# abcqmars/audio-visual-sepatation-in-visual-agnostic-situtation

Measured on AMD Instinct MI355X. Metric: mixtures/sec (train step, 2-src MUSIC shape), higher is better.
Workload: dtype f32; 1 GPU; full HIP path, AV train step: 2-source mix, batch 64/GPU (BASELINE configs[2] shape), 65535-sample waveforms -> HIP STFT 1022/256 -> 256x256 log-freq tiles, 3x224^2 frames/source, unet7+hidsep(sig)+resnet18dilated, BCE, SGD; f32 arithmetic; visual trunk on this library (no MIOpen kernel in the step); global_batch=64, parallelism=dp1

## Files before the change

### audio-visual-sepatation-in-visual-agnostic-situtation_amd/csrc/conv3x3.hip

```cpp
#include <stdlib.h>

#include "halo_kernel.h"
#include "conv_families.h"

__global__ void c3_pack_kernel(const float* __restrict__ w, float* __restrict__ out, int Cout, int Cin, int rows, int ld,
                               int mode) {
  long long i = (long long)blockIdx.x * blockDim.x + threadIdx.x;
  if (i >= (long long)rows * ld) return;
  int row = (int)(i / ld), col = (int)(i % ld);
  int parity = row & 1, q = row >> 1, tap = q % 9, ch = 2 * (q / 9) + parity;
  float v = 0.f;
  if (mode == 0) {
    if (ch < Cin && col < Cout) v = w[((long long)col * Cin + ch) * 9 + tap];
  } else {
    if (ch < Cout && col < Cin) v = w[((long long)ch * Cin + col) * 9 + (8 - tap)];
  }
  out[i] = v;
}

static bool c3_flat_enabled(int algo) { return !(algo & AVSEP_ALGO_NO_FLAT); }
static bool c3_flat(const avsep_conv_desc* d) {
  return !d->up2x && d->C0 == d->Cin && c3_flat_width(d->H, d->W, d->dil) > 0 && (long long)d->N * d->H * d->W < 0x7fffffffLL &&
         c3_flat_enabled(d->algo);
}
// ... 96 lines not shown
  } else {
    int per = Cout * 4, cls = row / per, rr = row % per;
    int parity = rr & 1, q = rr >> 1, tap = q % 4, ch = 2 * (q / 4) + parity;
    int ph = cls >> 1, pw = cls & 1, th = tap >> 1, tw = tap & 1;
    int kh = ph ? 2 - 2 * th : 3 - 2 * th, kw = pw ? 2 - 2 * tw : 3 - 2 * tw;
    if (ch < Cout && col < Cin) v = w[((long long)ch * Cin + col) * 16 + kh * 4 + kw];
  }
  out[i] = v;
}

bool c4_applicable(const avsep_conv_desc* d, int mode) {
  if (!(d->KH == 4 && d->KW == 4 && d->stride == 2 && d->pad == 1 && d->dil == 1) || d->up2x) return false;
  if (d->Wo < 16 || d->Ho < 4 || d->N > 65535) return false;
  if (mode == 0) return d->Cin % 2 == 0 && d->C0 % 2 == 0 && d->Cout >= 32;
  return d->Cout % 8 == 0 && d->Cin >= 32 && (d->H & 1) == 0 && (d->W & 1) == 0;
}
size_t c4_packed_floats(const avsep_conv_desc* d, int mode) {
  int rows = (mode == 0 ? d->Cin : d->Cout) * 16, ld = roundup(mode == 0 ? d->Cout : d->Cin, 128);
  return (size_t)rows * ld;
}
int c4_pack(const avsep_conv_desc* d, const float* w, float* packed, int mode, hipStream_t st) {
  int rows = (mode == 0 ? d->Cin : d->Cout) * 16, ld = roundup(mode == 0 ? d->Cout : d->Cin, 128);
  long long total = (long long)rows * ld;
  hipLaunchKernelGGL(c4_pack_kernel, dim3(cdiv(total, 256)), dim3(256), 0, st, w, packed, d->Cout, d->Cin, rows, ld, mode);
  AVSEP_LAUNCH_CHECK();
  return AVSEP_OK;
}

template <int KS_, int S_, int CK_>
static int c4_launch(C3Args& a, hipStream_t st) {
  const bool wide = a.Wo >= 32;
  a.tilesX = cdiv(a.Wo, wide ? 32 : 16);
  a.tilesY = cdiv(a.Ho, wide ? 4 : 8);
  const bool narrow = c3_narrow_rule(a.Cout, (long long)cdiv(a.Cout, 128) * a.tilesX * a.tilesY * c3_plan_n(a), false);
  a.gridM = cdiv(a.Cout, narrow ? 64 : 128);
  dim3 grid((unsigned)((long long)a.gridM * a.tilesX * a.tilesY * a.N));
  if (wide && !narrow) hipLaunchKernelGGL((conv3x3_kernel<4, 32, 128, false, KS_, S_, 1, CK_>), grid, dim3(256), 0, st, a);
  else if (wide) hipLaunchKernelGGL((conv3x3_kernel<4, 32, 64, false, KS_, S_, 1, CK_>), grid, dim3(256), 0, st, a);
  else if (!narrow) hipLaunchKernelGGL((conv3x3_kernel<8, 16, 128, false, KS_, S_, 1, CK_>), grid, dim3(256), 0, st, a);
  else hipLaunchKernelGGL((conv3x3_kernel<8, 16, 64, false, KS_, S_, 1, CK_>), grid, dim3(256), 0, st, a);
  AVSEP_LAUNCH_CHECK();
  return AVSEP_OK;
}

int c4_fwd(const avsep_conv_desc* d, const float* wp, const float* bias, float* y, double* stats, void*, size_t,
           hipStream_t st) {
  C3Args a{};
  a.N = d->N; a.planN = d->plan_n; a.algo = d->algo; a.Cin = d->Cin; a.H = d->H; a.W = d->W; a.Cout = d->Cout;
  a.C0 = d->C0; a.C1 = d->Cin - d->C0; a.act0 = d->act0; a.act1 = d->act1; a.up2x = 0;
  a.Hs = d->H; a.Ws = d->W;
  a.x0 = d->x0; a.x1 = d->x1; a.sc0 = d->scale0; a.sh0 = d->shift0; a.sc1 = d->scale1; a.sh1 = d->shift1;
  a.wp = wp; a.wp_ld = roundup(d->Cout, 128); a.out = y; a.bias = bias; a.stats = stats;
  a.Ho = d->Ho; a.Wo = d->Wo; a.padh = a.padw = 1; a.os = 1; a.ooh = a.oow = 0; a.OHs = d->Ho; a.OWs = d->Wo;
  return c4_launch<4, 2, 2>(a, st);
}

int c4_dgrad(const avsep_conv_desc* d, const float* wp, const float* dy, float* dx, const avsep_act_bwd*, void*, size_t,
             hipStream_t st) {
  const int ld = roundup(d->Cin, 128);
  for (int cls = 0; cls < 4; ++cls) {
    const int ph = cls >> 1, pw = cls & 1;
    C3Args a{};
    a.N = d->N; a.planN = d->plan_n; a.algo = d->algo; a.Cin = d->Cout; a.H = d->Ho; a.W = d->Wo; a.Cout = d->Cin;
    a.C0 = d->Cout; a.C1 = 0; a.Hs = d->Ho; a.Ws = d->Wo;
    a.x0 = dy; a.wp = wp + (size_t)cls * d->Cout * 4 * ld; a.wp_ld = ld; a.out = dx;
    a.Ho = d->H / 2; a.Wo = d->W / 2; a.padh = ph ? 0 : 1; a.padw = pw ? 0 : 1;
    a.os = 2; a.ooh = ph; a.oow = pw; a.OHs = d->H; a.OWs = d->W;
    int rc = c4_launch<2, 1, 8>(a, st);
    if (rc) return rc;
  }
  return AVSEP_OK;
}

int c1x4_stft_fwd(const float* xt, const float* wp, float* out, int R, int NH, int hop, int cout, int frames,
                  hipStream_t st) {
  C3Args a{};
  a.N = 1; a.Cin = hop; a.H = R; a.W = NH; a.Cout = cout;
  a.C0 = hop; a.C1 = 0; a.Hs = R; a.Ws = NH;
  a.x0 = xt; a.wp = wp; a.wp_ld = roundup(cout, 128); a.out = out;
  a.Ho = R; a.Wo = frames; a.padh = a.padw = 0; a.os = 1; a.ooh = a.oow = 0; a.OHs = R; a.OWs = frames;
  a.tilesX = cdiv(frames, 32); a.tilesY = cdiv(R, 4); a.gridM = cdiv(cout, 128);
  dim3 grid((unsigned)((long long)a.gridM * a.tilesX * a.tilesY));
  hipLaunchKernelGGL((conv3x3_kernel<4, 32, 128, false, 1, 1, 1, 4, 1, 4>), grid, dim3(256), 0, st, a);
  AVSEP_LAUNCH_CHECK();
  return AVSEP_OK;
}

struct W3Args {
  int N, Cin, H, W, Cout, Ho, Wo;
  int C0, C1, act0, act1, up2x, Hs, Ws;
  float rh, rw;
  const float *x0, *x1, *sc0, *sh0, *sc1, *sh1;
  const float* dy;
  float* out;
  int tilesX, tilesY, gridM, gridC, tiles_per_split;
  int tapmajor;
};

constexpr int W3_CC = 32;

__device__ __forceinline__ float w3_src(const W3Args& a, int n, int c, int hs, int ws) {
  float v;
  if (c < a.C0) {
    v = a.x0[(((long long)n * a.C0 + c) * a.Hs + hs) * a.Ws + ws];
    if (a.sc0) v = fmaf(v, a.sc0[c], a.sh0[c]);
    v = act_apply(v, a.act0);
  } else {
    int c1 = c - a.C0;
    v = a.x1[(((long long)n * a.C1 + c1) * a.Hs + hs) * a.Ws + ws];
    if (a.sc1) v = fmaf(v, a.sc1[c1], a.sh1[c1]);
    v = act_apply(v, a.act1);
  }
  return v;
}

template <int TH, int TW, int PW, int MAXT, int TAP0, int NTAP, int DIL = 1, int S = 1>
__device__ __forceinline__ void w3_mfma_tile(const float* Ap, const float* Bp, f32x16 (&acc)[MAXT]) {
#pragma unroll 1
  for (int py = 0; py < TH; ++py) {
    const float* ar = Ap + py * TW;
    const float* br = Bp + py * S * PW;
    float av[2], bv[2][NTAP];
    av[0] = ar[0];
#pragma unroll
    for (int j = 0; j < NTAP; ++j) bv[0][j] = br[(((TAP0 + j) / 3) * PW + (TAP0 + j) % 3) * DIL];
#pragma unroll 4
    for (int px = 0; px < TW; px += 2) {
      const int cur = (px >> 1) & 1;
      if (px + 2 < TW) {
        av[cur ^ 1] = ar[px + 2];
#pragma unroll
        for (int j = 0; j < NTAP; ++j) bv[cur ^ 1][j] = br[(((TAP0 + j) / 3) * PW + (TAP0 + j) % 3) * DIL + (px + 2) * S];
      }
      __builtin_amdgcn_sched_barrier(0);
#pragma unroll
      for (int j = 0; j < NTAP; ++j) acc[j] = __builtin_amdgcn_mfma_f32_32x32x2f32(av[cur], bv[cur][j], acc[j], 0, 0, 0);
      __builtin_amdgcn_sched_barrier(0);
    }
  }
}

template <int TH, int TW, bool UP2X, int BM, int DIL = 1, bool A2 = false, int S = 1>
__global__ __launch_bounds__(512, 2) void wgrad3x3_kernel(W3Args a) {
  static_assert(!(UP2X && DIL != 1), "the fused upsample path is undilated");
  static_assert(S == 1 || (DIL == 1 && !UP2X), "stride 2: plain 3x3 / pad 1");
  constexpr int NPIX = TH * TW, PH = (TH - 1) * S + 2 * DIL + 1, PW = (TW - 1) * S + 2 * DIL + 1;
  constexpr int PS = (PH * PW) | 1;
  constexpr int LDA = NPIX + 1;
  constexpr int NT = 512;
  constexpr int NP = W3_CC * PH * PW, PE = (NP + NT - 1) / NT;
  constexpr int NA4 = BM * NPIX / 4, AE = NA4 / NT;
  static_assert(NA4 % NT == 0, "A tile must split evenly");
  __shared__ float smem[2 * W3_CC * PS + 2 * BM * LDA];
  float (*Ps)[W3_CC * PS] = reinterpret_cast<float (*)[W3_CC * PS]>(smem);
  float (*As)[BM * LDA] = reinterpret_cast<float (*)[BM * LDA]>(smem + 2 * W3_CC * PS);

  const int tid = threadIdx.x, lane = tid & 63, wave = tid >> 6, li = lane & 31, lk = lane >> 5;
  const int t_ = xcd_remap(blockIdx.x, gridDim.x), per_split_ = a.gridM * a.gridC;
  const int split = t_ / per_split_, lin_ = t_ % per_split_;
  const int mt = lin_ % a.gridM, ct = lin_ / a.gridM;
  const int m0 = mt * BM, c0 = ct * W3_CC;
  const int tiles_img = a.tilesX * a.tilesY, tiles_all = tiles_img * a.N;
  const int t_begin = split * a.tiles_per_split, t_end = min(tiles_all, t_begin + a.tiles_per_split);
  const long long HW = (long long)a.Ho * a.Wo;

  constexpr int RB = BM / 32, MAXT = (BM == 128) ? 5 : 3;
// ... 268 lines not shown
```

### audio-visual-sepatation-in-visual-agnostic-situtation_amd/csrc/conv_families.h

```cpp
#pragma once
#include "common.h"

typedef bool conv_applicable_fn(const avsep_conv_desc* d, int mode);
typedef size_t conv_packed_floats_fn(const avsep_conv_desc* d, int mode);
typedef int conv_pack_fn(const avsep_conv_desc* d, const float* w, float* packed, int mode, hipStream_t st);
typedef size_t conv_workspace_fn(const avsep_conv_desc* d, int mode);
typedef void conv_variant_fn(const avsep_conv_desc* d, int mode, char* buf, size_t cap);
typedef int conv_fwd_fn(const avsep_conv_desc* d, const float* wp, const float* bias, float* y, double* stats, void* ws,
                        size_t ws_bytes, hipStream_t st);
typedef int conv_dgrad_fn(const avsep_conv_desc* d, const float* wp, const float* dy, float* dx, const avsep_act_bwd* e,
                          void* ws, size_t ws_bytes, hipStream_t st);
typedef int conv_wgrad_fn(const avsep_conv_desc* d, const float* dy, float* dw, float* dbias, float* ws, hipStream_t st);

static inline int igemm_packed_ld(const avsep_conv_desc* d, int mode) { return roundup(mode == 0 ? d->Cout : d->Cin, 128); }

int splitk_combine(const float* ws, long long slab, int S, const avsep_conv_desc* d, const float* bias, float* y, double* stats,
                   hipStream_t st);
int reduce_slabs(const float* ws, float* out, long long n, int S, hipStream_t st);
int reduce_slabs_strided(const float* ws, float* out, long long n, int S, long long stride, hipStream_t st);

conv_applicable_fn smallco_applicable;  conv_workspace_fn smallco_workspace_bytes;  conv_fwd_fn smallco_fwd;  conv_wgrad_fn smallco_wgrad;
conv_applicable_fn smallci_applicable;  conv_packed_floats_fn smallci_packed_floats;  conv_pack_fn smallci_pack;  conv_dgrad_fn smallci_dgrad;

conv_applicable_fn head_applicable;  conv_workspace_fn head_workspace_bytes;  conv_fwd_fn head_fwd;  conv_wgrad_fn head_wgrad;
size_t head_dgrad_workspace_floats(const avsep_conv_desc* d);
int head_dgrad(const avsep_conv_desc* d, const float* w, const float* dy, float* g0, float* g1, const float* mean1,
               const float* invstd1, double* bstats1, int acc0, float* ws, hipStream_t st);

conv_applicable_fn bf_applicable;  conv_packed_floats_fn bf_packed_floats;  conv_pack_fn bf_pack;  conv_workspace_fn bf_workspace_bytes;
conv_fwd_fn bf_fwd;  conv_dgrad_fn bf_dgrad;  conv_variant_fn bf_variant;
bool bf_out_b16(const avsep_conv_desc* d, int mode);

conv_applicable_fn w4_applicable;  conv_packed_floats_fn w4_packed_floats;  conv_pack_fn w4_pack;
conv_fwd_fn w4_fwd;  conv_dgrad_fn w4_dgrad;  conv_variant_fn w4_variant;

conv_applicable_fn wn_applicable;  conv_packed_floats_fn wn_packed_floats;  conv_pack_fn wn_pack;  conv_fwd_fn wn_fwd;  conv_dgrad_fn wn_dgrad;

conv_applicable_fn c3_applicable;  conv_packed_floats_fn c3_packed_floats;  conv_pack_fn c3_pack;
conv_fwd_fn c3_fwd;  conv_dgrad_fn c3_dgrad;  conv_variant_fn c3_variant;
conv_applicable_fn c4_applicable;  conv_packed_floats_fn c4_packed_floats;  conv_pack_fn c4_pack;
conv_fwd_fn c4_fwd;  conv_dgrad_fn c4_dgrad;  conv_variant_fn c4_variant;
conv_applicable_fn w3_applicable;  conv_workspace_fn w3_workspace_bytes;  conv_wgrad_fn w3_wgrad;
void c3_variant_text(int M, int Ho, int Wo, long long planN, bool flat, bool quantise, char* buf, size_t cap);
int w3_reduce(const float* ws, float* dw, long long P, int splits, hipStream_t st);
int c1x4_stft_fwd(const float* xt, const float* wp, float* out, int R, int NH, int hop, int cout, int frames, hipStream_t st);

struct C3Args;
int c3_flat_width(int H, int W, int dil);
int c3_flat_launch(C3Args& a, int dil, hipStream_t st);

conv_applicable_fn cm_applicable;  conv_packed_floats_fn cm_packed_floats;  conv_pack_fn cm_pack;
conv_fwd_fn cm_fwd;  conv_dgrad_fn cm_dgrad;  conv_variant_fn cm_variant;

conv_applicable_fn wbn_applicable;  conv_workspace_fn wbn_workspace_bytes;  conv_wgrad_fn wbn_wgrad;  conv_variant_fn wbn_variant;
int b16_channel_sum(const void* x, int N, int C, int HW, double* acc, float* out, hipStream_t st);

conv_applicable_fn x4_applicable;  conv_workspace_fn x4_workspace_bytes;  conv_wgrad_fn x4_wgrad;  conv_variant_fn x4_variant;

conv_applicable_fn ww_applicable;  conv_workspace_fn ww_workspace_bytes;  conv_wgrad_fn ww_wgrad;
conv_applicable_fn w4d_applicable;  conv_workspace_fn w4d_workspace_bytes;  conv_wgrad_fn w4d_wgrad;

conv_applicable_fn scw_applicable;  conv_workspace_fn scw_workspace_bytes;  conv_wgrad_fn scw_wgrad;
```

### audio-visual-sepatation-in-visual-agnostic-situtation_amd/csrc/halo_kernel.h

```cpp
#pragma once
#include "common.h"

struct C3Args {
  int N, Cin, H, W, Cout;
  int C0, C1, act0, act1, up2x, Hs, Ws;
  float rh, rw;
  const float *x0, *x1, *sc0, *sh0, *sc1, *sh1;
  const float* wp;
  int wp_ld;
  float* out;
  const float* bias;
  double* stats;
  int tilesX, tilesY, gridM;
  int Ho, Wo;
  int padh, padw;
  int os, ooh, oow;
  int OHs, OWs;
  int kts;
  long long slab;
  int planN;
  int algo;
  int out16;
  int xs2;
};
static inline long long c3_plan_n(const C3Args& a) { return a.planN > 0 ? a.planN : a.N; }
static inline bool c3_narrow_rule(int cout, long long wg128, bool quantise) {
  return cout <= 64 || wg128 < 384 || (quantise && wg128 < 1024 && wg128 * 5 < ((wg128 + 255) / 256) * 256 * 4);
}

constexpr int C3_CK = 4;

__device__ __forceinline__ float c3_src(const C3Args& a, int n, int c, int hs, int ws) {
  float v;
  if (c < a.C0) {
    v = a.x0[(((long long)n * a.C0 + c) * a.Hs + hs) * a.Ws + ws];
    if (a.sc0) v = fmaf(v, a.sc0[c], a.sh0[c]);
    v = act_apply(v, a.act0);
  } else {
    int c1 = c - a.C0;
    v = a.x1[(((long long)n * a.C1 + c1) * a.Hs + hs) * a.Ws + ws];
    if (a.sc1) v = fmaf(v, a.sc1[c1], a.sh1[c1]);
    v = act_apply(v, a.act1);
  }
  return v;
}

template <int TH, int TW, int BM, bool UP2X, int KS = 3, int S = 1, int DIL = 1, int CK = 4, int KH_ = KS, int KW_ = KS,
          int FW = 0, bool ZF = false>
__global__ __launch_bounds__(256) void conv3x3_kernel(C3Args a) {
  constexpr bool FLAT = FW > 0;
  static_assert(!ZF || (!FLAT && !UP2X), "zero fill: rectangular tiles");
  static_assert(!FLAT || (S == 1 && !UP2X && (KH_ & 1) && (KW_ & 1)), "flat tiles: stride 1, odd taps, no fused upsample");
  constexpr int NT = KH_ * KW_, C3_KT = CK * NT, C3_CK = CK;
  constexpr int PADH = DIL * (KH_ - 1) / 2, PADW = DIL * (KW_ - 1) / 2;
  constexpr int F_NR = (FW + 126 + (FLAT ? FW : 1)) / (FLAT ? FW : 1);
  constexpr int F_NC = 127 / (FLAT ? FW * FW : 1) + 1;
  constexpr int PH = FLAT ? F_NR + F_NC * PADH + 2 * PADH : (TH - 1) * S + (KH_ - 1) * DIL + 1;
  constexpr int PWR = FLAT ? FW + 2 * PADW : (TW - 1) * S + (KW_ - 1) * DIL + 1;
  constexpr int PW = (S == 2) ? (PWR + 1) / 2 * 2 : PWR, PWH = PW / 2, PS = PH * PW;
  constexpr int LDA = BM + 4;
  constexpr int NPATCH = C3_CK * PS;
  constexpr int PE = (NPATCH + 255) / 256;
  constexpr int A4 = BM / 4, NA4 = C3_KT * A4, AE = (NA4 + 255) / 256;
  constexpr int WTM = BM / 2, TM = WTM / 32;
  __shared__ __attribute__((aligned(16))) float As[2][C3_KT][LDA];
  __shared__ float Ps[2][NPATCH];

  const int tid = threadIdx.x, lane = tid & 63, wave = tid >> 6;
  const int wm = wave >> 1, wn = wave & 1, li = lane & 31, lk = lane >> 5;
  int t = xcd_remap(blockIdx.x, gridDim.x);
  const int mt = t % a.gridM; t /= a.gridM;
  const int tx = t % a.tilesX; t /= a.tilesX;
  const int ty = t % a.tilesY;
  const int n = t / a.tilesY;
  const int h0 = ty * TH, w0 = tx * TW, m0 = mt * BM;
  const int f_HW = a.H * a.W, f_Hp = a.H + PADH, f_P = a.N * f_HW;
  const int p0 = tx * 128;
  const int vr0 = FLAT ? (p0 / f_HW) * f_Hp + (p0 % f_HW) / FW : 0;

  const bool has0 = a.sc0 != nullptr, has1 = a.sc1 != nullptr;
  const long long sHW = (long long)a.Hs * a.Ws;
  f32x4 areg[AE];
  const float* aptr[AE];
  int a_lds[AE];
#pragma unroll
  for (int e = 0; e < AE; ++e) {
    int idx = min(tid + 256 * e, NA4 - 1);
    int row = idx / A4, c4 = idx % A4;
    aptr[e] = a.wp + (long long)row * a.wp_ld + m0 + c4 * 4;
    a_lds[e] = row * LDA + c4 * 4;
  }
  const long long a_step = (long long)C3_KT * a.wp_ld;

  constexpr int NRAW = UP2X ? 4 : 1;
  float praw[PE][NRAW], psc[PE], psh[PE], plh[UP2X ? PE : 1], plw[UP2X ? PE : 1];
  const float* pptr[PE][NRAW];
  long long poff1[PE][NRAW];
  int p_cc[PE];
  int p_lds[S == 2 ? PE : 1];
  unsigned pok = 0;
#pragma unroll
  for (int e = 0; e < PE; ++e) {
    int idx = min(tid + 256 * e, NPATCH - 1);
    int cc = idx / PS, r = (idx % PS) / PW, col = idx % PW;
    int gh = h0 * S - a.padh + r, gw = w0 * S - a.padw + col;
    int ne = n;
    if constexpr (FLAT) {
      const int vr = vr0 - PADH + r;
      ne = vr >= 0 ? vr / f_Hp : a.N;
      gh = vr >= 0 ? vr % f_Hp : -1;
      gw = col - PADW;
      if (ne >= a.N) { ne = a.N - 1; gh = -1; }
    }
    if constexpr (S == 2) p_lds[e] = cc * PS + r * PW + (col & 1) * PWH + (col >> 1);
    bool ok = (PE * 256 == NPATCH || tid + 256 * e < NPATCH) && (unsigned)gh < (unsigned)a.H && (unsigned)gw < (unsigned)a.W;
    int ghc = min(max(gh, 0), a.H - 1), gwc = min(max(gw, 0), a.W - 1);
    long long o[NRAW];
    if constexpr (!UP2X) {
      o[0] = ((long long)ghc * a.Ws + gwc) << a.xs2;
    } else {
      float fh = a.rh * (float)ghc, fw = a.rw * (float)gwc;
      int hh0 = (int)fh, ww0 = (int)fw;
      int hh1 = hh0 + (hh0 < a.Hs - 1), ww1 = ww0 + (ww0 < a.Ws - 1);
      plh[e] = fh - (float)hh0;
      plw[e] = fw - (float)ww0;
      o[0] = (long long)hh0 * a.Ws + ww0; o[1] = (long long)hh0 * a.Ws + ww1;
      o[2] = (long long)hh1 * a.Ws + ww0; o[3] = (long long)hh1 * a.Ws + ww1;
    }
#pragma unroll
    for (int q = 0; q < NRAW; ++q) {
      pptr[e][q] = a.x0 + ((long long)ne * a.C0 + cc) * sHW + o[q];
      poff1[e][q] = ((long long)ne * a.C1 + cc) * sHW + o[q];
    }
    p_cc[e] = cc;
    pok |= (unsigned)ok << e;
  }
  const long long p_step = (long long)C3_CK * sHW;
  const int kt_switch = a.C0 / C3_CK;
  bool cur_has = has0;
  const float *scp = a.sc0, *shp = a.sh0;

  auto issue = [&](int kt) __attribute__((always_inline)) {
    if (kt == kt_switch && a.C1 > 0) {
#pragma unroll
      for (int e = 0; e < PE; ++e)
#pragma unroll
        for (int q = 0; q < NRAW; ++q) pptr[e][q] = a.x1 + poff1[e][q];
      cur_has = has1;
      scp = a.sc1;
      shp = a.sh1;
    }
#pragma unroll
    for (int e = 0; e < AE; ++e) {
      areg[e] = *reinterpret_cast<const f32x4*>(aptr[e]);
      aptr[e] += a_step;
    }
#pragma unroll
    for (int e = 0; e < PE; ++e) {
#pragma unroll
      for (int q = 0; q < NRAW; ++q) {
        praw[e][q] = *pptr[e][q];
        pptr[e][q] += p_step;
      }
      if (cur_has) {
        psc[e] = scp[p_cc[e]];
        psh[e] = shp[p_cc[e]];
      }
    }
    if (cur_has) {
      scp += C3_CK;
      shp += C3_CK;
    }
// ... 155 lines not shown
```

### audio-visual-sepatation-in-visual-agnostic-situtation_amd/csrc/stft.hip

```cpp
#include "common.h"
#include "conv_families.h"
#include "stft_parts.h"

static inline int bins_of(int n_fft) { return n_fft / 2 + 1; }

extern "C" size_t avsep_stft_basis_floats(int32_t n_fft, int32_t inverse) {
  if (n_fft < 2 || (n_fft & 1)) return 0;
  int b2 = 2 * bins_of(n_fft);
  return inverse ? (size_t)roundup(b2, 32) * roundup(n_fft, 128) : (size_t)roundup(n_fft, 32) * roundup(b2, 128);
}

__global__ void stft_basis_kernel(int n_fft, int bins, int rows, int ld, int inverse, float* __restrict__ out) {
  long long i = (long long)blockIdx.x * blockDim.x + threadIdx.x;
  if (i >= (long long)rows * ld) return;
  int row = (int)(i / ld), col = (int)(i % ld);
  int n = inverse ? col : row, m = inverse ? row : col;
  float v = 0.f;
  if (n < n_fft && m < 2 * bins) {
    int bin = m < bins ? m : m - bins;
    double win = 0.5 - 0.5 * cos(2.0 * M_PI * (double)n / (double)n_fft);
    long long prod = ((long long)bin * n) % n_fft;
    double ang = 2.0 * M_PI * (double)prod / (double)n_fft;
    double tr = (m < bins) ? cos(ang) : -sin(ang);
    if (inverse) {
// ... 1 lines not shown
      if (m >= bins && (bin == 0 || bin == n_fft / 2)) ck = 0.0;
      tr *= ck / (double)n_fft;
    }
    v = (float)(win * tr);
  }
  out[i] = v;
}

extern "C" int avsep_stft_basis(int32_t n_fft, float* fwd_basis, float* inv_basis, avsep_stream_t stream) {
  if (n_fft < 2 || (n_fft & 1)) return AVSEP_ERR_ARG;
  int bins = bins_of(n_fft), b2 = 2 * bins;
  if (fwd_basis) {
    int rows = roundup(n_fft, 32), ld = roundup(b2, 128);
    hipLaunchKernelGGL(stft_basis_kernel, dim3(cdiv((long long)rows * ld, 256)), dim3(256), 0, (hipStream_t)stream, n_fft,
                       bins, rows, ld, 0, fwd_basis);
    AVSEP_LAUNCH_CHECK();
  }
  if (inv_basis) {
    int rows = roundup(b2, 32), ld = roundup(n_fft, 128);
    hipLaunchKernelGGL(stft_basis_kernel, dim3(cdiv((long long)rows * ld, 256)), dim3(256), 0, (hipStream_t)stream, n_fft,
                       bins, rows, ld, 1, inv_basis);
    AVSEP_LAUNCH_CHECK();
  }
  return AVSEP_OK;
}

__global__ __launch_bounds__(256) void stft_pad_kernel(const float* __restrict__ wav, int L, int pad, int reflect,
                                                       float* __restrict__ out) {
  const int r = blockIdx.y, Lp = L + 2 * pad;
  for (int i = blockIdx.x * 256 + threadIdx.x; i < Lp; i += gridDim.x * 256) {
    int j = i - pad;
    float v = 0.f;
    if (j >= 0 && j < L) v = wav[(long long)r * L + j];
    else if (reflect) {
      if (j < 0) j = -j;
      if (j >= L) j = 2 * (L - 1) - j;
      if (j >= 0 && j < L) v = wav[(long long)r * L + j];
    }
    out[(long long)r * Lp + i] = v;
  }
}

__global__ __launch_bounds__(256) void stft_pad_t_kernel(const float* __restrict__ wav, int L, int pad, int reflect, int hop,
                                                         int R, int NH, float* __restrict__ xt) {
  extern __shared__ float tile[];
  const int r = blockIdx.y, j0 = blockIdx.x * 32, Lp = L + 2 * pad, ldt = hop + 1;
  for (int i = threadIdx.x; i < 32 * hop; i += 256) {
    const int jj = i / hop, c = i % hop, pos = (j0 + jj) * hop + c;
    float v = 0.f;
    if (pos < Lp) {
      int s = pos - pad;
      if (s >= 0 && s < L) v = wav[(long long)r * L + s];
      else if (reflect) {
        if (s < 0) s = -s;
        if (s >= L) s = 2 * (L - 1) - s;
        if (s >= 0 && s < L) v = wav[(long long)r * L + s];
      }
    }
    tile[jj * ldt + c] = v;
  }
  __syncthreads();
  for (int i = threadIdx.x; i < 32 * hop; i += 256) {
    const int c = i / 32, jj = i % 32;
    if (j0 + jj < NH) xt[((long long)c * R + r) * NH + j0 + jj] = tile[jj * ldt + c];
  }
}

__global__ void stft_basis_repack_kernel(const float* __restrict__ basis, int n_fft, int hop, int ntap, int ld,
                                         float* __restrict__ out) {
  long long i = (long long)blockIdx.x * blockDim.x + threadIdx.x;
  if (i >= (long long)hop * ntap * ld) return;
  const int row = (int)(i / ld), col = (int)(i % ld);
  const int par = row & 1, q = row >> 1, j = q % ntap, c = 2 * (q / ntap) + par, k = hop * j + c;
  out[i] = k < n_fft ? basis[(long long)k * ld + col] : 0.f;
}

__global__ __launch_bounds__(256) void stft_magphase_kernel(const float* __restrict__ spec, int bins, int frames, int R,
                                                            int co_major, float* __restrict__ mag,
                                                            float* __restrict__ phase) {
  const int r = blockIdx.y;
  const long long n = (long long)bins * frames;
  for (long long i = (long long)blockIdx.x * 256 + threadIdx.x; i < n; i += (long long)gridDim.x * 256) {
    float a, b;
    if (co_major) {
      const long long m = i / frames, f = i % frames;
      a = spec[(m * R + r) * frames + f];
      b = spec[((bins + m) * R + r) * frames + f];
    } else {
      a = spec[(long long)r * 2 * n + i];
      b = spec[(long long)r * 2 * n + n + i];
    }
    mag[(long long)r * n + i] = sqrtf(a * a + b * b);
    if (phase) phase[(long long)r * n + i] = atan2f(b, a);
  }
}


static bool stft_fast(int R, int L, int n_fft, int hop) {
  return n_fft > 3 * hop && n_fft <= 4 * hop && (hop & 3) == 0 && hop <= 1024 && 1 + L / hop >= 32 && R >= 1;
}
extern "C" size_t avsep_stft_workspace_bytes(int32_t R, int32_t L, int32_t n_fft, int32_t hop) {
  if (R <= 0 || L <= 0 || n_fft < 2 || hop <= 0) return 0;
  size_t frames = 1 + L / hop;
  size_t spec = (size_t)R * 2 * bins_of(n_fft) * frames;
  if (stft_fast(R, L, n_fft, hop))
    return ((size_t)hop * R * (frames + 3) + (size_t)hop * 4 * roundup(2 * bins_of(n_fft), 128) + spec) * sizeof(float);
  return ((size_t)R * (L + n_fft) + spec) * sizeof(float);
}

bool stft_fast_path(int R, int L, int n_fft, int hop) { return stft_fast(R, L, n_fft, hop); }

int stft_repack_basis(const float* basis, int n_fft, int hop, float* wp, hipStream_t st) {
  const int ld = roundup(2 * bins_of(n_fft), 128);
  hipLaunchKernelGGL(stft_basis_repack_kernel, dim3(cdiv((long long)hop * 4 * ld, 256)), dim3(256), 0, st, basis, n_fft, hop,
                     4, ld, wp);
  AVSEP_LAUNCH_CHECK();
  return AVSEP_OK;
}

int stft_pad_gemm(const float* wav, int R, int L, int n_fft, int hop, int reflect, const float* basis, float* stage, float* spec,
                  hipStream_t st) {
  const int pad = n_fft / 2, Lp = L + 2 * pad, bins = bins_of(n_fft), frames = 1 + L / hop;
  if (stft_fast(R, L, n_fft, hop)) {
    const int NH = frames + 3;
    hipLaunchKernelGGL(stft_pad_t_kernel, dim3(cdiv(NH, 32), R), dim3(256), (size_t)32 * (hop + 1) * sizeof(float), st, wav, L,
                       pad, reflect, hop, R, NH, stage);
    AVSEP_LAUNCH_CHECK();
    return c1x4_stft_fwd(stage, basis, spec, R, NH, hop, 2 * bins, frames, st);
  }
  hipLaunchKernelGGL(stft_pad_kernel, dim3(min(cdiv(Lp, 256), 1024), R), dim3(256), 0, st, wav, L, pad, reflect, stage);
  AVSEP_LAUNCH_CHECK();
  avsep_conv_desc d{};
  d.N = R; d.Cin = 1; d.H = 1; d.W = Lp; d.Cout = 2 * bins; d.Ho = 1; d.Wo = frames;
  d.KH = 1; d.KW = n_fft; d.stride = hop; d.pad = 0; d.dil = 1; d.C0 = 1; d.x0 = stage;
  return avsep_conv2d_fwd(&d, basis, nullptr, spec, nullptr, nullptr, 0, (avsep_stream_t)st);
}

int istft_gemm(const float* spec, int R, int n_fft, int frames, const float* inv_basis, float* td, hipStream_t st) {
  avsep_conv_desc d{};
  d.N = R; d.Cin = 2 * bins_of(n_fft); d.H = 1; d.W = frames; d.Cout = n_fft; d.Ho = 1; d.Wo = frames;
  d.KH = 1; d.KW = 1; d.stride = 1; d.pad = 0; d.dil = 1; d.C0 = d.Cin; d.x0 = spec;
  return avsep_conv2d_fwd(&d, inv_basis, nullptr, td, nullptr, nullptr, 0, (avsep_stream_t)st);
}

extern "C" int avsep_stft_mag(const float* wav, int32_t R, int32_t L, int32_t n_fft, int32_t hop, int32_t reflect,
                              const float* basis, float* mag, float* phase, void* workspace, size_t workspace_bytes,
                              avsep_stream_t stream) {
  if (!wav || !basis || !mag || R <= 0 || R > 65535 || L <= n_fft / 2 || n_fft < 2 || (n_fft & 1) || hop <= 0)
    return AVSEP_ERR_ARG;
  if (!workspace || workspace_bytes < avsep_stft_workspace_bytes(R, L, n_fft, hop)) return AVSEP_ERR_WORKSPACE;
  const int pad = n_fft / 2, Lp = L + 2 * pad, bins = bins_of(n_fft), frames = 1 + L / hop;
  hipStream_t st = (hipStream_t)stream;
  const bool fast = stft_fast(R, L, n_fft, hop);
  float* stage = (float*)workspace;
  const float* b = basis;
  float* spec;
  if (fast) {
    float* wp = stage + (size_t)hop * R * (frames + 3);
    spec = wp + (size_t)hop * 4 * roundup(2 * bins, 128);
    int rc = stft_repack_basis(basis, n_fft, hop, wp, st);
    if (rc) return rc;
    b = wp;
  } else {
    spec = stage + (size_t)R * Lp;
  }
  int rc = stft_pad_gemm(wav, R, L, n_fft, hop, reflect, b, stage, spec, st);
  if (rc) return rc;
  long long n = (long long)bins * frames;
  hipLaunchKernelGGL(stft_magphase_kernel, dim3((int)min((n + 255) / 256, (long long)1024), R), dim3(256), 0, st, spec, bins,
                     frames, R, fast ? 1 : 0, mag, phase);
  AVSEP_LAUNCH_CHECK();
  return AVSEP_OK;
}

__global__ __launch_bounds__(256) void istft_spec_kernel(const float* __restrict__ mag, const float* __restrict__ phase,
                                                         long long n, float* __restrict__ spec) {
  const int r = blockIdx.y;
  for (long long i = (long long)blockIdx.x * 256 + threadIdx.x; i < n; i += (long long)gridDim.x * 256) {
    float m = mag[(long long)r * n + i], p = phase[(long long)r * n + i];
    float s, c;
    sincosf(p, &s, &c);
    spec[(long long)r * 2 * n + i] = m * c;
    spec[(long long)r * 2 * n + n + i] = m * s;
  }
}

__global__ __launch_bounds__(256) void istft_ola_kernel(const float* __restrict__ td, int n_fft, int hop, int frames,
                                                        int out_len, float* __restrict__ wav) {
  const int r = blockIdx.y, pad = n_fft / 2;
  const float* p = td + (long long)r * n_fft * frames;
  for (int t = blockIdx.x * 256 + threadIdx.x; t < out_len; t += gridDim.x * 256) {
    int g = t + pad;
    int f_hi = min(frames - 1, g / hop), f_lo = max(0, (g - n_fft + hop) / hop);
    float acc = 0.f, wss = 0.f;
    for (int f = f_lo; f <= f_hi; ++f) {
      int n = g - f * hop;
      if (n < 0 || n >= n_fft) continue;
      float w = 0.5f - 0.5f * cosf(2.f * (float)M_PI * (float)n / (float)n_fft);
      acc += p[(long long)n * frames + f];
      wss += w * w;
    }
    wav[(long long)r * out_len + t] = wss > 1.17549435e-38f ? acc / wss : acc;
  }
}

extern "C" size_t avsep_istft_workspace_bytes(int32_t R, int32_t n_fft, int32_t frames) {
  if (R <= 0 || n_fft < 2 || frames <= 0) return 0;
  return ((size_t)R * 2 * bins_of(n_fft) * frames + (size_t)R * n_fft * frames) * sizeof(float);
}

extern "C" int avsep_istft(const float* mag, const float* phase, int32_t R, int32_t n_fft, int32_t hop, int32_t frames,
                           const float* inv_basis, float* wav, int32_t out_len, void* workspace, size_t workspace_bytes,
                           avsep_stream_t stream) {
  if (!mag || !phase || !inv_basis || !wav || R <= 0 || R > 65535 || n_fft < 2 || (n_fft & 1) || hop <= 0 || frames <= 0)
    return AVSEP_ERR_ARG;
  if (out_len <= 0 || out_len > hop * (frames - 1)) return AVSEP_ERR_ARG;
  if (!workspace || workspace_bytes < avsep_istft_workspace_bytes(R, n_fft, frames)) return AVSEP_ERR_WORKSPACE;
  const int bins = bins_of(n_fft);
  float* spec = (float*)workspace;
  float* td = spec + (size_t)R * 2 * bins * frames;
  hipStream_t st = (hipStream_t)stream;
  long long n = (long long)bins * frames;
  hipLaunchKernelGGL(istft_spec_kernel, dim3((int)min((n + 255) / 256, (long long)1024), R), dim3(256), 0, st, mag, phase, n,
                     spec);
  AVSEP_LAUNCH_CHECK();
  int rc = istft_gemm(spec, R, n_fft, frames, inv_basis, td, st);
  if (rc) return rc;
  hipLaunchKernelGGL(istft_ola_kernel, dim3(min(cdiv(out_len, 256), 1024), R), dim3(256), 0, st, td, n_fft, hop, frames,
                     out_len, wav);
  AVSEP_LAUNCH_CHECK();
  return AVSEP_OK;
}
```

### audio-visual-sepatation-in-visual-agnostic-situtation_amd/models/vision_hip.py

```python
import torch

from .. import kernels as K
from .. import lib
from ..lib import ACT_NONE, ACT_RELU
from .audio_net import ParamGrads, _bn_back, _bn_run


def _geom(conv):
    k, s, p, d = conv.kernel_size, conv.stride, conv.padding, conv.dilation
    if k[0] != k[1] or s[0] != s[1] or p[0] != p[1] or d[0] != d[1]:
        raise lib.AvsepError("the HIP visual trunk needs square conv geometry")
    return k[0], s[0], p[0], d[0]


def _w(conv):
    return conv.weight.detach().contiguous()


def _conv(src, conv, aff=None):
    k, s, p, d = _geom(conv)
    if aff is None:
        return K.Conv(src, conv.out_channels, k, s, p, d)
    return K.Conv(src, conv.out_channels, k, s, p, d, sc0=aff[0], sh0=aff[1], act0=ACT_RELU)


def _conv_bn(src, conv, bn, training, aff=None):
    cv = _conv(src, conv, aff)
    st = K.zeros_stats(conv.out_channels, src) if training else None
    y = cv.fwd(cv.pack(_w(conv), 0), None, st)
    return cv, y, _bn_run(bn, st, K.per_channel(y), training, src)


def blocks_of(features):
    return [b for i in (4, 5, 6, 7) for b in features[i]]


def param_list(net):
    return list(net.features.parameters()) + list(net.fc.parameters())


_S2D_INDEX = {}


def _stem_s2d_weight(w):
    Co, Cc = w.shape[:2]
    key = (Cc, w.device)
    if key not in _S2D_INDEX:
        idx = torch.zeros((16, 4, 4), dtype=torch.long)
        ok = torch.zeros((16, 4, 4), dtype=torch.bool)
        for q in range(4 * Cc):
            c, dy, dx = q % Cc, (q // Cc) >> 1, (q // Cc) & 1
            for a in range(4):
                for b in range(4):
                    kh, kw = 2 * a + dy - 1, 2 * b + dx - 1
                    if 0 <= kh <= 6 and 0 <= kw <= 6:
                        idx[q, a, b], ok[q, a, b] = (c * 7 + kh) * 7 + kw, True
        _S2D_INDEX[key] = (idx.to(w.device).reshape(-1), ok.to(w.device).reshape(1, 16, 4, 4))
    idx, ok = _S2D_INDEX[key]
    return (w.reshape(Co, -1)[:, idx].reshape(Co, 16, 4, 4) * ok).contiguous()


def _stem_s2d_weight_grad(dw2, Cc):
    Co = dw2.shape[0]
    key = ("inv", Cc, dw2.device)
    if key not in _S2D_INDEX:
        inv = torch.zeros((Cc, 7, 7), dtype=torch.long)
        for q in range(4 * Cc):
            c, dy, dx = q % Cc, (q // Cc) >> 1, (q // Cc) & 1
            for a in range(4):
                for b in range(4):
                    kh, kw = 2 * a + dy - 1, 2 * b + dx - 1
                    if 0 <= kh <= 6 and 0 <= kw <= 6:
                        inv[c, kh, kw] = (q * 4 + a) * 4 + b
        _S2D_INDEX[key] = inv.to(dw2.device).reshape(-1)
    return dw2.reshape(Co, -1)[:, _S2D_INDEX[key]].reshape(Co, Cc, 7, 7)


def _stem_is_s2d(conv, x):
    return (conv.kernel_size == (7, 7) and conv.stride == (2, 2) and conv.padding == (3, 3) and conv.dilation == (1, 1)
            and conv.in_channels <= 4 and x.shape[2] % 2 == 0 and x.shape[3] % 2 == 0)


def stem_forward(f, x, training):
    S = {"x": x}
    if _stem_is_s2d(f[0], x):
        S["cv0"] = _conv(x, f[0])
        cs = K.Conv(K.space_to_depth2(x), f[0].out_channels, 4, 1, 0)
        S["cs"] = cs
        st = K.zeros_stats(f[0].out_channels, x) if training else None
        S["y0"] = cs.fwd(cs.pack(_stem_s2d_weight(_w(f[0])), 0), None, st)
        S["bn0"] = _bn_run(f[1], st, K.per_channel(S["y0"]), training, x)
    else:
        S["cv0"], S["y0"], S["bn0"] = _conv_bn(x, f[0], f[1], training)
    z, S["idx"] = K.maxpool3x3s2(S["y0"], S["bn0"][0], S["bn0"][1], ACT_RELU)
    return S, z


def block_forward(blk, z, training):
    R = {"mod": blk, "z": z}
    R["cv1"], R["y1"], R["bn1"] = _conv_bn(z, blk.conv1, blk.bn1, training)
    if K.get_precision() == "f32":
        a1 = K.affine_act(R["y1"], R["bn1"][0], R["bn1"][1], None, ACT_RELU)
        R["cv2"], R["y2"], R["bn2"] = _conv_bn(a1, blk.conv2, blk.bn2, training)
    else:
        R["cv2"], R["y2"], R["bn2"] = _conv_bn(R["y1"], blk.conv2, blk.bn2, training, aff=R["bn1"])
    if blk.downsample is not None:
        R["cvd"], R["yd"], R["bnd"] = _conv_bn(z, blk.downsample[0], blk.downsample[1], training)
        out = K.affine_act(R["y2"], R["bn2"][0], R["bn2"][1], R["yd"], ACT_RELU, R["bnd"][0], R["bnd"][1])
    else:
        out = K.affine_act(R["y2"], R["bn2"][0], R["bn2"][1], R["z"], ACT_RELU)
    return R, out


def fc_forward(fc, z):
    cvf = _conv(z, fc)
    bias = fc.bias.detach() if fc.bias is not None else None
    return cvf, cvf.fwd(cvf.pack(_w(fc), 0), bias, None, out_b16=False)


def trunk_forward(net, x, training):
    S, z = stem_forward(net.features, x, training)
    S["blocks"] = []
    for blk in blocks_of(net.features):
        R, z = block_forward(blk, z, training)
        S["blocks"].append(R)
    S["cvf"], out = fc_forward(net.fc, z)
    return S, out


def _relu_bn_back(grads, g, y, bnrow, bn_mod, res=None, rs=None, rh=None, g2=None):
    bst = K.zeros_stats(K.channels(y), y)
    g = K.affine_act_bwd_(g, y, bnrow[0], bnrow[1], res, None, bnrow[2], bnrow[3], ACT_RELU, bst, res_scale=rs, res_shift=rh,
                          dz2=g2)
    return g, _bn_back(grads, bn_mod, bnrow, bst, K.per_channel(y))


def fc_backward(fc, cvf, dout, grads):
    grads.wgrad(cvf, fc.weight, dout, fc.bias)
    return cvf.dgrad(cvf.pack(_w(fc), 1), dout)


def block_backward(R, g, grads, g2=None):
    blk = R["mod"]
    ds = blk.downsample is not None
    bnd = R.get("bnd")
    g, pqr2 = _relu_bn_back(grads, g, R["y2"], R["bn2"], blk.bn2, res=R["yd"] if ds else R["z"],
                            rs=bnd[0] if ds else None, rh=bnd[1] if ds else None, g2=g2)
    dy2 = K.bn_bwd_apply_(g, R["y2"], pqr2, fresh=True)
    grads.wgrad(R["cv2"], blk.conv2.weight, dy2)
    if K.get_precision() == "f32" and not K.is_b16(R["y1"]):
        bn1 = R["bn1"]
        bst1 = K.zeros_stats(K.channels(R["y1"]), R["y1"])
        da = R["cv2"].dgrad_act(R["cv2"].pack(_w(blk.conv2), 1), dy2, R["y1"], bn1[0], bn1[1], bn1[2], bn1[3], ACT_RELU, bst1)
        pqr1 = _bn_back(grads, blk.bn1, bn1, bst1, K.per_channel(R["y1"]))
        del dy2
    else:
        da = R["cv2"].dgrad(R["cv2"].pack(_w(blk.conv2), 1), dy2)
        del dy2
        da, pqr1 = _relu_bn_back(grads, da, R["y1"], R["bn1"], blk.bn1)
    da = K.bn_bwd_apply_(da, R["y1"], pqr1)
    grads.wgrad(R["cv1"], blk.conv1.weight, da)
    dz = R["cv1"].dgrad(R["cv1"].pack(_w(blk.conv1), 1), da)
    del da
    if ds:
        bst = K.zeros_stats(K.channels(g), g)
        g = K.affine_act_bwd_(g, R["yd"], None, None, None, None, bnd[2], bnd[3], ACT_NONE, bst, stats_only=True)
        pqrd = _bn_back(grads, blk.downsample[1], bnd, bst, K.per_channel(g))
        g = K.bn_bwd_apply_(g, R["yd"], pqrd)
        grads.wgrad(R["cvd"], blk.downsample[0].weight, g)
        return dz, R["cvd"].dgrad(R["cvd"].pack(_w(blk.downsample[0]), 1), g)
    return dz, g


# ... 48 lines not shown
```

Before: 874.8 mixtures/s.

## Fold STFT via even/odd symmetry into smaller GEMM; trim stem s2d channel padding

Adds a folded STFT path for odd-half n_fft. A prep kernel windows the frames and combines symmetric sample pairs into four even/odd quadrant inputs. These feed a batched GEMM (N=4 weight slabs via a new wp_ns stride) with about a quarter of the basis, replacing the full DFT basis GEMM. Magphase gets a new index mode to undo the interleaved bin order. Separately, the f32 visual stem's space-to-depth conv now uses 4*Cin channels instead of 16, cutting padded work, which risks hitting a less tuned kernel path.

```diff
diff --git a/audio-visual-sepatation-in-visual-agnostic-situtation_amd/csrc/conv3x3.hip b/audio-visual-sepatation-in-visual-agnostic-situtation_amd/csrc/conv3x3.hip
--- a/audio-visual-sepatation-in-visual-agnostic-situtation_amd/csrc/conv3x3.hip
+++ b/audio-visual-sepatation-in-visual-agnostic-situtation_amd/csrc/conv3x3.hip
@@ -202,6 +202,22 @@
   a.tilesX = cdiv(frames, 32); a.tilesY = cdiv(R, 4); a.gridM = cdiv(cout, 128);
   dim3 grid((unsigned)((long long)a.gridM * a.tilesX * a.tilesY));
   hipLaunchKernelGGL((conv3x3_kernel<4, 32, 128, false, 1, 1, 1, 4, 1, 4>), grid, dim3(256), 0, st, a);
+  AVSEP_LAUNCH_CHECK();
+  return AVSEP_OK;
+}
+
+int stft_folded_gemm(const float* F, const float* wp, float* out, int R, int frames, int Kp, int M, hipStream_t st) {
+  C3Args a{};
+  a.N = 4; a.Cin = Kp; a.H = R; a.W = frames; a.Cout = M;
+  a.C0 = Kp; a.C1 = 0; a.Hs = R; a.Ws = frames;
+  a.x0 = F; a.wp = wp; a.wp_ld = roundup(M, 128); a.wp_ns = (long long)Kp * a.wp_ld; a.out = out;
+  a.Ho = R; a.Wo = frames; a.padh = a.padw = 0; a.os = 1; a.ooh = a.oow = 0; a.OHs = R; a.OWs = frames;
+  a.tilesX = cdiv(frames, 32); a.tilesY = cdiv(R, 4);
+  const bool narrow = M <= 64;
+  a.gridM = cdiv(M, narrow ? 64 : 128);
+  dim3 grid((unsigned)((long long)a.gridM * a.tilesX * a.tilesY * a.N));
+  if (narrow) hipLaunchKernelGGL((conv3x3_kernel<4, 32, 64, false, 3, 1, 1, 16, 1, 1>), grid, dim3(256), 0, st, a);
+  else hipLaunchKernelGGL((conv3x3_kernel<4, 32, 128, false, 3, 1, 1, 16, 1, 1>), grid, dim3(256), 0, st, a);
   AVSEP_LAUNCH_CHECK();
   return AVSEP_OK;
 }
diff --git a/audio-visual-sepatation-in-visual-agnostic-situtation_amd/csrc/conv_families.h b/audio-visual-sepatation-in-visual-agnostic-situtation_amd/csrc/conv_families.h
--- a/audio-visual-sepatation-in-visual-agnostic-situtation_amd/csrc/conv_families.h
+++ b/audio-visual-sepatation-in-visual-agnostic-situtation_amd/csrc/conv_families.h
@@ -44,6 +44,7 @@
 void c3_variant_text(int M, int Ho, int Wo, long long planN, bool flat, bool quantise, char* buf, size_t cap);
 int w3_reduce(const float* ws, float* dw, long long P, int splits, hipStream_t st);
 int c1x4_stft_fwd(const float* xt, const float* wp, float* out, int R, int NH, int hop, int cout, int frames, hipStream_t st);
+int stft_folded_gemm(const float* F, const float* wp, float* out, int R, int frames, int Kp, int M, hipStream_t st);
 
 struct C3Args;
 int c3_flat_width(int H, int W, int dil);
diff --git a/audio-visual-sepatation-in-visual-agnostic-situtation_amd/csrc/halo_kernel.h b/audio-visual-sepatation-in-visual-agnostic-situtation_amd/csrc/halo_kernel.h
--- a/audio-visual-sepatation-in-visual-agnostic-situtation_amd/csrc/halo_kernel.h
+++ b/audio-visual-sepatation-in-visual-agnostic-situtation_amd/csrc/halo_kernel.h
@@ -22,6 +22,7 @@
   int algo;
   int out16;
   int xs2;
+  long long wp_ns;
 };
 static inline long long c3_plan_n(const C3Args& a) { return a.planN > 0 ? a.planN : a.N; }
 static inline bool c3_narrow_rule(int cout, long long wg128, bool quantise) {
@@ -87,7 +88,7 @@
   for (int e = 0; e < AE; ++e) {
     int idx = min(tid + 256 * e, NA4 - 1);
     int row = idx / A4, c4 = idx % A4;
-    aptr[e] = a.wp + (long long)row * a.wp_ld + m0 + c4 * 4;
+    aptr[e] = a.wp + n * a.wp_ns + (long long)row * a.wp_ld + m0 + c4 * 4;
     a_lds[e] = row * LDA + c4 * 4;
   }
   const long long a_step = (long long)C3_KT * a.wp_ld;
diff --git a/audio-visual-sepatation-in-visual-agnostic-situtation_amd/csrc/stft.hip b/audio-visual-sepatation-in-visual-agnostic-situtation_amd/csrc/stft.hip
--- a/audio-visual-sepatation-in-visual-agnostic-situtation_amd/csrc/stft.hip
+++ b/audio-visual-sepatation-in-visual-agnostic-situtation_amd/csrc/stft.hip
@@ -107,7 +107,11 @@
   const long long n = (long long)bins * frames;
   for (long long i = (long long)blockIdx.x * 256 + threadIdx.x; i < n; i += (long long)gridDim.x * 256) {
     float a, b;
-    if (co_major) {
+    if (co_major == 2) {
+      const long long m = i / frames, f = i % frames, hb = bins / 2, row = (m & 1) * hb + (m >> 1);
+      a = spec[(row * R + r) * frames + f];
+      b = spec[((2 * hb + row) * R + r) * frames + f];
+    } else if (co_major) {
       const long long m = i / frames, f = i % frames;
       a = spec[(m * R + r) * frames + f];
       b = spec[((bins + m) * R + r) * frames + f];
@@ -121,13 +125,81 @@
 }
 
 
+static inline int fold_pairs(int n_fft) { return (n_fft / 2 - 1) / 2; }
+static inline int fold_k(int n_fft) { return roundup(1 + fold_pairs(n_fft), 16); }
+
+__global__ void stft_fold_basis_kernel(int n_fft, int P, int M, int Kp, int ld, float* __restrict__ out) {
+  long long i = (long long)blockIdx.x * blockDim.x + threadIdx.x;
+  if (i >= 4LL * Kp * ld) return;
+  const int col = (int)(i % ld), j = (int)((i / ld) % Kp), q = (int)(i / ((long long)ld * Kp));
+  float v = 0.f;
+  if (col < M) {
+    if (j == 0) v = q == 0 ? 1.f : q == 1 ? -1.f : 0.f;
+    else if (j <= P) {
+      const int k = 2 * col + (q & 1);
+      long long prod = ((long long)k * j) % n_fft;
+      double ang = 2.0 * M_PI * (double)prod / (double)n_fft;
+      v = (float)(q < 2 ? cos(ang) : -sin(ang));
+    }
+  }
+  out[i] = v;
+}
+
+__global__ __launch_bounds__(256) void stft_fold_kernel(const float* __restrict__ wav, int L, int n_fft, int hop, int reflect,
+                                                        int R, int frames, int Kp, float* __restrict__ F) {
+  extern __shared__ float sm[];
+  const int h = n_fft / 2, P = (h - 1) / 2, pad = h, Lp = L + 2 * pad;
+  const int ns = 31 * hop + n_fft;
+  float* xs = sm;
+  float* win = sm + ns + ns / hop + 1;
+  const int r = blockIdx.y, f0 = blockIdx.x * 32, tid = threadIdx.x;
+  for (int i = tid; i <= h; i += 256) win[i] = (float)(0.5 - 0.5 * cos(2.0 * M_PI * (double)i / (double)n_fft));
+  for (int i = tid; i < ns; i += 256) {
+    const long long pos = (long long)f0 * hop + i;
+    float v = 0.f;
+    if (pos < Lp) {
+      int s = (int)pos - pad;
+      if (s >= 0 && s < L) v = wav[(long long)r * L + s];
+      else if (reflect) {
+        if (s < 0) s = -s;
+        if (s >= L) s = 2 * (L - 1) - s;
+        if (s >= 0 && s < L) v = wav[(long long)r * L + s];
+      }
+    }
+    xs[i + i / hop] = v;
+  }
+  __syncthreads();
+  const int fl = tid & 31, f = f0 + fl, base = fl * (hop + 1);
+  auto X = [&](int n) __attribute__((always_inline)) {
+    return xs[base + n + (n >= hop) + (n >= 2 * hop) + (n >= 3 * hop)];
+  };
+  const size_t qs = (size_t)Kp * R * frames;
+  for (int j = tid >> 5; j < Kp; j += 8) {
+    float v0 = 0.f, v1 = 0.f, v2 = 0.f, v3 = 0.f;
+    if (j == 0) {
+      v0 = v1 = win[h] * X(h);
+    } else if (j <= P) {
+      const float a = X(j), b = X(n_fft - j), c = X(h - j), d = X(h + j), wm = win[j], wh = win[h - j];
+      const float e1 = wm * (a + b), e2 = wh * (c + d), o1 = wm * (a - b), o2 = wh * (c - d);
+      v0 = e1 + e2; v1 = e1 - e2; v2 = o1 - o2; v3 = o1 + o2;
+    }
+    if (f < frames) {
+      float* o = F + ((size_t)j * R + r) * frames + f;
+      o[0] = v0; o[qs] = v1; o[2 * qs] = v2; o[3 * qs] = v3;
+    }
+  }
+}
+
 static bool stft_fast(int R, int L, int n_fft, int hop) {
   return n_fft > 3 * hop && n_fft <= 4 * hop && (hop & 3) == 0 && hop <= 1024 && 1 + L / hop >= 32 && R >= 1;
 }
+static bool stft_folded(int R, int L, int n_fft, int hop) { return stft_fast(R, L, n_fft, hop) && n_fft % 4 == 2 && hop <= 256; }
 extern "C" size_t avsep_stft_workspace_bytes(int32_t R, int32_t L, int32_t n_fft, int32_t hop) {
   if (R <= 0 || L <= 0 || n_fft < 2 || hop <= 0) return 0;
   size_t frames = 1 + L / hop;
   size_t spec = (size_t)R * 2 * bins_of(n_fft) * frames;
+  if (stft_folded(R, L, n_fft, hop))
+    return (4 * (size_t)fold_k(n_fft) * (R * frames + roundup(bins_of(n_fft) / 2, 128)) + spec) * sizeof(float);
   if (stft_fast(R, L, n_fft, hop))
     return ((size_t)hop * R * (frames + 3) + (size_t)hop * 4 * roundup(2 * bins_of(n_fft), 128) + spec) * sizeof(float);
   return ((size_t)R * (L + n_fft) + spec) * sizeof(float);
@@ -176,6 +248,25 @@
   if (!workspace || workspace_bytes < avsep_stft_workspace_bytes(R, L, n_fft, hop)) return AVSEP_ERR_WORKSPACE;
   const int pad = n_fft / 2, Lp = L + 2 * pad, bins = bins_of(n_fft), frames = 1 + L / hop;
   hipStream_t st = (hipStream_t)stream;
+  if (stft_folded(R, L, n_fft, hop)) {
+    const int Kp = fold_k(n_fft), P = fold_pairs(n_fft), M = bins / 2, ld = roundup(M, 128);
+    float* F = (float*)workspace;
+    float* wp = F + 4 * (size_t)Kp * R * frames;
+    float* spec = wp + 4 * (size_t)Kp * ld;
+    hipLaunchKernelGGL(stft_fold_basis_kernel, dim3(cdiv(4LL * Kp * ld, 256)), dim3(256), 0, st, n_fft, P, M, Kp, ld, wp);
+    AVSEP_LAUNCH_CHECK();
+    const int ns = 31 * hop + n_fft;
+    hipLaunchKernelGGL(stft_fold_kernel, dim3(cdiv(frames, 32), R), dim3(256), (size_t)(ns + ns / hop + 1 + pad + 1) * sizeof(float),
+                       st, wav, L, n_fft, hop, reflect, R, frames, Kp, F);
+    AVSEP_LAUNCH_CHECK();
+    int rc = stft_folded_gemm(F, wp, spec, R, frames, Kp, M, st);
+    if (rc) return rc;
+    long long n = (long long)bins * frames;
+    hipLaunchKernelGGL(stft_magphase_kernel, dim3((int)min((n + 255) / 256, (long long)1024), R), dim3(256), 0, st, spec, bins,
+                       frames, R, 2, mag, phase);
+    AVSEP_LAUNCH_CHECK();
+    return AVSEP_OK;
+  }
   const bool fast = stft_fast(R, L, n_fft, hop);
   float* stage = (float*)workspace;
   const float* b = basis;
diff --git a/audio-visual-sepatation-in-visual-agnostic-situtation_amd/models/vision_hip.py b/audio-visual-sepatation-in-visual-agnostic-situtation_amd/models/vision_hip.py
--- a/audio-visual-sepatation-in-visual-agnostic-situtation_amd/models/vision_hip.py
+++ b/audio-visual-sepatation-in-visual-agnostic-situtation_amd/models/vision_hip.py
@@ -42,12 +42,12 @@
 _S2D_INDEX = {}
 
 
-def _stem_s2d_weight(w):
+def _stem_s2d_weight(w, cp=16):
     Co, Cc = w.shape[:2]
-    key = (Cc, w.device)
+    key = (Cc, cp, w.device)
     if key not in _S2D_INDEX:
-        idx = torch.zeros((16, 4, 4), dtype=torch.long)
-        ok = torch.zeros((16, 4, 4), dtype=torch.bool)
+        idx = torch.zeros((cp, 4, 4), dtype=torch.long)
+        ok = torch.zeros((cp, 4, 4), dtype=torch.bool)
         for q in range(4 * Cc):
             c, dy, dx = q % Cc, (q // Cc) >> 1, (q // Cc) & 1
             for a in range(4):
@@ -55,9 +55,9 @@
                     kh, kw = 2 * a + dy - 1, 2 * b + dx - 1
                     if 0 <= kh <= 6 and 0 <= kw <= 6:
                         idx[q, a, b], ok[q, a, b] = (c * 7 + kh) * 7 + kw, True
-        _S2D_INDEX[key] = (idx.to(w.device).reshape(-1), ok.to(w.device).reshape(1, 16, 4, 4))
+        _S2D_INDEX[key] = (idx.to(w.device).reshape(-1), ok.to(w.device).reshape(1, cp, 4, 4))
     idx, ok = _S2D_INDEX[key]
-    return (w.reshape(Co, -1)[:, idx].reshape(Co, 16, 4, 4) * ok).contiguous()
+    return (w.reshape(Co, -1)[:, idx].reshape(Co, cp, 4, 4) * ok).contiguous()
 
 
 def _stem_s2d_weight_grad(dw2, Cc):
@@ -81,14 +81,19 @@
             and conv.in_channels <= 4 and x.shape[2] % 2 == 0 and x.shape[3] % 2 == 0)
 
 
+def _stem_cp(conv):
+    return 4 * conv.in_channels if K.get_precision() == "f32" else 16
+
+
 def stem_forward(f, x, training):
     S = {"x": x}
     if _stem_is_s2d(f[0], x):
         S["cv0"] = _conv(x, f[0])
-        cs = K.Conv(K.space_to_depth2(x), f[0].out_channels, 4, 1, 0)
+        cp = _stem_cp(f[0])
+        cs = K.Conv(K.space_to_depth2(x, cp), f[0].out_channels, 4, 1, 0)
         S["cs"] = cs
         st = K.zeros_stats(f[0].out_channels, x) if training else None
-        S["y0"] = cs.fwd(cs.pack(_stem_s2d_weight(_w(f[0])), 0), None, st)
+        S["y0"] = cs.fwd(cs.pack(_stem_s2d_weight(_w(f[0]), cp), 0), None, st)
         S["bn0"] = _bn_run(f[1], st, K.per_channel(S["y0"]), training, x)
     else:
         S["cv0"], S["y0"], S["bn0"] = _conv_bn(x, f[0], f[1], training)
```

Measured after the change: 882.7 mixtures/s (median of 6 runs). No clear change (+0.9%).
